# THGLab/NewtonNet

Hardware: AMD Instinct MI355X
Metric: atom-steps/sec (energy+force) on batched MD17 aspirin (higher is better)
Workload: dtype f32; 1 GPU; MD17 aspirin batched inference, 1024 conformers x 21 atoms per GPU, fp32, energy+force, neighbor list included (BASELINE.json configs[1]); 2 independent step(s) in flight per GPU; atoms_per_gpu=21504, weights=seed0, distinct_batches=4, steps_in_flight=2, parallelism=1 independent shard(s), no data-path collective

## Files before the change

### newtonnet_amd/csrc/common.h

```cpp
#pragma once
#include <hip/hip_runtime.h>
#include <stdint.h>

#include "../../include/newtonnet_hip.h"

#if (defined(EDGE_ABL_SELF) || defined(EDGE_ABL_PAIR) || defined(EDGE_ABL_TABLE) || defined(EDGE_ABL_STORE) ||              \
     defined(EDGE_ABL_NO_TABLE) || defined(EDGE_ABL_HALF_TABLE) || defined(EDGE_ABL_NOTAB) || defined(EDGE_ABL_NOMJ) || defined(MLPS_ABL_NO_H) || defined(NS_ABL_NO_Q) || defined(NS_ABL_HOT_W) || defined(MLPS_ABL_X) || defined(ABL_NO_SILU) || defined(ABL_NO_STORE) ||                  \
     (defined(LIN_ABLATE_NO_LOAD) && LIN_ABLATE_NO_LOAD) || (defined(LIN_ABLATE_NO_STORE) && LIN_ABLATE_NO_STORE) ||         \
     (defined(LIN_ABLATE_NO_MFMA) && LIN_ABLATE_NO_MFMA) || (defined(LIN_ABLATE_NO_LDS) && LIN_ABLATE_NO_LDS)) &&            \
    !defined(NNHIP_TOOLING)
#error "ablation switches produce wrong results: build through csrc/build.sh (it marks the library with -DNNHIP_TOOLING)"
#endif

#define NF NNHIP_F
#define NB NNHIP_NB
#define WAVE 64
#ifndef FT_G
#define FT_G 3072
#endif
#define FT_ROWS (FT_G + 8)
#define FT_ZERO_ROW (FT_G + 3)
#define FT_PLANE ((size_t)FT_ROWS * NNHIP_F)

typedef float f32x16 __attribute__((ext_vector_type(16)));
// ... 299 lines not shown
struct WeightImageJobs {
  const float* src[WIMG_MAX_JOBS];
  char* dst[WIMG_MAX_JOBS];
  int fmt;
};
enum { IMG_UPDATE = 0, IMG_NODE0, IMG_NODE2, IMG_UPDATE_T, IMG_NODE0_T, IMG_NODE2_T, IMG_EQ1_0, IMG_EQ1_2, IMG_EQ2_0, IMG_EQ2_2,
       IMG_EQ1_0_T, IMG_EQ1_2_T, IMG_EQ2_0_T, IMG_EQ2_2_T, IMG_PER_LAYER };
enum { IMG_HEAD0 = 0, IMG_HEAD2, IMG_HEAD0_T, IMG_HEAD2_T, IMG_HEAD_COUNT };
struct NodeImages {
  const char *Wu, *W0, *W2;
  const char *W2T, *W0T, *WuT;
};
int launch_weight_images(const float* const* src, char* const* dst, int n, hipStream_t s, int fmt = WIMG_FMT_SPLIT_F16);
int launch_node_fwd_split(const NodeFwdArgs& a, const NodeImages& im, hipStream_t s);
int launch_node_bwd_split(const NodeBwdArgs& a, const NodeImages& im, hipStream_t s);
int launch_mlp_wide_split(int mode, bool accum, const MlpArgs& a, hipStream_t s);
int launch_mlp_wide_pair_split(int mode, const MlpPair& P, hipStream_t s);
int launch_lin_wide_split(const float* X, int ldx, const char* img, float* Y, int ldy, int M, bool acc, hipStream_t s);
bool split_products_enabled();

static inline int cdiv(long a, long b) { return (int)((a + b - 1) / b); }
```

### newtonnet_amd/csrc/edge.hip

```cpp
#include <stdlib.h>

#include <type_traits>

#include "common.h"

#include "edge_common.h"

template <int WPR>
__global__ void __launch_bounds__(64 * EDGE_ROWS)
msg_fwd_kernel(const float* __restrict__ m, const int2* __restrict__ xg, const float* __restrict__ table,
               const int* __restrict__ row_ptr, const int* __restrict__ col, const int* __restrict__ pid,
               const float* __restrict__ a_in, float* __restrict__ msg , float* __restrict__ a_mid,
               int n_atoms) {
  __shared__ float4 comb[EDGE_COMB_SIZE(WPR, 1)];
  int part;
  const int i_ = wave_row_split<WPR>(gridDim.x, part);
  const bool active = i_ < n_atoms;
  if (WPR == 1 && !active) return;
  const int i = active ? i_ : 0;
  const int lane = threadIdx.x & 63;
  const int c4 = 4 * (lane & 31);
  const bool hi = lane >= 32;
  const float4 mi = ld4(m + (size_t)i * NF + c4);
  float4 acc = make_float4(0.f, 0.f, 0.f, 0.f);
// ... 344 lines not shown
      float4 eps, deps;
      filter_value_deriv(table, ABL_G(gx.x), c4, fw, eps, deps);
      const float gxs = half_sum_top(dot4(mul4(mul4(G, mi), mj), deps));
      if ((lane & 31) == 31) g_x[eh] = gxs;
      if (NEED_GM) acc = fma4(mul4(G, eps), mj, acc);
    }
  }
  if (NEED_GM) {
    acc = add4(acc, upper_half(acc));
    float4 a1[1] = {acc};
    row_combine<WPR, 1>(a1, comb, part, lane);
    if (active && part == 0 && !hi) st4(g_m + (size_t)i * NF + c4, a1[0]);
  }
}

template <bool NEED_GM>
__global__ void __launch_bounds__(64 * FM_WAVES)
msg_bwd_mol_kernel(const float* __restrict__ g_msg , const float* __restrict__ g_a, const float* __restrict__ m,
                   const int2* __restrict__ xg, const float* __restrict__ table, const int* __restrict__ mol_ptr,
                   const int* __restrict__ row_ptr, const int* __restrict__ col, const int* __restrict__ pid,
                   float* __restrict__ g_m, float* __restrict__ g_x, int n_mol, const int* __restrict__ pair_ptr) {
  __shared__ __attribute__((aligned(16))) float ml[NNHIP_MOL_STAGE_MAX * NF];
  __shared__ __attribute__((aligned(16))) float gl[NNHIP_MOL_STAGE_MAX * NF];
  __shared__ int s_next;
  const int b = xcd_tile(blockIdx.x, gridDim.x);
  if (b >= n_mol) return;
  const int a0 = mol_ptr[b], n = mol_ptr[b + 1] - a0;
  const bool staged = n <= NNHIP_MOL_STAGE_MAX;
  if (staged) {
    const float4* sm = reinterpret_cast<const float4*>(m + (size_t)a0 * NF);
    const float4* sg = reinterpret_cast<const float4*>(g_a + (size_t)a0 * NF);
    for (int t = threadIdx.x; t < n * (NF / 4); t += 64 * FM_WAVES) {
      reinterpret_cast<float4*>(ml)[t] = sm[t];
      reinterpret_cast<float4*>(gl)[t] = sg[t];
    }
  }
// ... 43 lines not shown
        const float4 mj = node(ml, m, j), gaj = node(gl, g_a, j);
        const float4 G = add4(add4(ld4(g_msg + p * NF + c4), gai), gaj);
        const FilterW fw = filter_weights(__int_as_float(gx.y));
        float4 eps, deps;
        filter_value_deriv(table, gx.x, c4, fw, eps, deps);
        const float gxs = half_sum_top(dot4(mul4(mul4(G, mi), mj), deps));
        if ((lane & 31) == 31) g_x[eh] = gxs;
        if (NEED_GM) acc = fma4(mul4(G, eps), mj, acc);
      }
    }
    if (NEED_GM) {
      acc = add4(acc, upper_half(acc));
      if (!hi) st4(g_m + (size_t)i * NF + c4, acc);
    }
  }
}

__global__ void __launch_bounds__(256)
edge_gd_kernel(const float* __restrict__ g_x , const float* __restrict__ g_u ,
               const float* __restrict__ geo, int n_edges, int n_layers, float inv_rc, float* __restrict__ g_d ) {
  const int e = blockIdx.x * blockDim.x + threadIdx.x;
  if (e >= n_edges) return;
  float gx = 0.f, gu0 = 0.f, gu1 = 0.f, gu2 = 0.f;
  for (int l = 0; l < n_layers; ++l) {
    gx += g_x[(size_t)l * n_edges + e];
    const float4 v = reinterpret_cast<const float4*>(g_u)[(size_t)l * n_edges + e];
    gu0 += v.x;
    gu1 += v.y;
    gu2 += v.z;
  }
// ... 318 lines not shown
  static const size_t v = getenv("NNHIP_EDGE_LDS") ? (size_t)atol(getenv("NNHIP_EDGE_LDS")) : 0;
  return v;
}

static bool mol_kernels_pay(int n_atoms, int n_mol) {
  static const int min_mol = getenv("NNHIP_MOL_KERNELS_MIN") ? atoi(getenv("NNHIP_MOL_KERNELS_MIN")) : 640;
  return n_mol >= min_mol && (long)n_atoms <= (long)n_mol * NNHIP_MOL_STAGE_MAX && (long)n_atoms >= 8L * n_mol;
}

void edge_config(int* small_atoms, int* mol_min, int* wpr , int* mol_forms ) {
  *small_atoms = getenv("NNHIP_EDGE_SMALL_ATOMS") ? atoi(getenv("NNHIP_EDGE_SMALL_ATOMS")) : EDGE_SMALL_ATOMS;
  *mol_min = getenv("NNHIP_MOL_KERNELS_MIN") ? atoi(getenv("NNHIP_MOL_KERNELS_MIN")) : 640;
  wpr[0] = EDGE_WPR_MSG_FWD, wpr[1] = EDGE_WPR_FORCE_FWD, wpr[2] = EDGE_WPR_FORCE_BWD, wpr[3] = EDGE_WPR_MSG_BWD;
  auto off = [](const char* name) { return getenv(name) && atoi(getenv(name)) == 0; };
  *mol_forms = (off("NNHIP_FORCE_FWD_MOL") ? 0 : 1) | (off("NNHIP_MSG_BWD_MOL") ? 0 : 2) | (off("NNHIP_FORCE_DIRECT_MOL") ? 0 : 4) |
               (off("NNHIP_HEAD_OUT_MOL") ? 0 : 8);
}

int launch_msg_fwd(const float* m, const int* xg, const float* table, const int* row_ptr, const int* col,
                   const int* pid, const float* a_in, float* msg, float* a_mid, int n_atoms, hipStream_t s) {
  ScopedTimer t0(TC_EDGE, s);
  ScopedTimer t1(TC_EDGE_FWD_MSG, s);
  EDGE_LAUNCH(msg_fwd_kernel, EDGE_WPR_MSG_FWD, m, reinterpret_cast<const int2*>(xg), table, row_ptr, col, pid, a_in, msg, a_mid, n_atoms);
  LAUNCH_CHECK();
  return 0;
}

int launch_force_fwd(bool has_f, const float* phi1, const float* phi2, const float* geo, const int* row_ptr,
                     const int* col, const int* pid, const float* f_in, float* f_out, int n_atoms, const int* xg,
                     hipStream_t s, const int* pair_ptr, const int* mol_ptr, int n_mol) {
  ScopedTimer t0(TC_EDGE, s);
// ... 18 lines not shown
                     float* g_fin, int n_atoms, const int* xg, hipStream_t s, const int* pair_ptr, const int* rev) {
  ScopedTimer t0(TC_EDGE, s);
  ScopedTimer t1(TC_EDGE_BWD_FORCE, s);
  static const bool owner_off = getenv("NNHIP_FORCE_BWD_OWNER_GU") && atoi(getenv("NNHIP_FORCE_BWD_OWNER_GU")) == 0;
  if (owner_off) rev = nullptr;
  if (has_f)
    EDGE_LAUNCH_B(force_bwd_kernel, true, EDGE_WPR_FORCE_BWD, gf, phi1, phi2, geo, row_ptr, col, pid, f_in, g_h12, g_u, g_fin, n_atoms, reinterpret_cast<const int2*>(xg), pair_ptr, rev);
  else
    EDGE_LAUNCH_B(force_bwd_kernel, false, EDGE_WPR_FORCE_BWD, gf, phi1, phi2, geo, row_ptr, col, pid, f_in, g_h12, g_u, g_fin, n_atoms, reinterpret_cast<const int2*>(xg), pair_ptr, rev);
  LAUNCH_CHECK();
  return 0;
}

int launch_msg_bwd(const float* g_msg, const float* g_a, const float* m, const int* xg, const float* table,
                   const int* row_ptr, const int* col, const int* pid, float* g_m, float* g_x, int n_atoms,
                   bool need_gm, hipStream_t s, const int* pair_ptr, const int* mol_ptr, int n_mol) {
  ScopedTimer t0(TC_EDGE, s);
  ScopedTimer t1(TC_EDGE_BWD_MSG, s);
  static const bool mol_off = getenv("NNHIP_MSG_BWD_MOL") && atoi(getenv("NNHIP_MSG_BWD_MOL")) == 0;
  if (mol_ptr && pair_ptr && mol_kernels_pay(n_atoms, n_mol) && !mol_off) {
    if (need_gm)
      msg_bwd_mol_kernel<true><<<n_mol, 64 * FM_WAVES, 0, s>>>(g_msg, g_a, m, reinterpret_cast<const int2*>(xg), table, mol_ptr, row_ptr,
                                                              col, pid, g_m, g_x, n_mol, pair_ptr);
    else
      msg_bwd_mol_kernel<false><<<n_mol, 64 * FM_WAVES, 0, s>>>(g_msg, g_a, m, reinterpret_cast<const int2*>(xg), table, mol_ptr, row_ptr,
                                                               col, pid, g_m, g_x, n_mol, pair_ptr);
    LAUNCH_CHECK();
    return 0;
  }
  if (need_gm)
    EDGE_LAUNCH_B(msg_bwd_kernel, true, EDGE_WPR_MSG_BWD, g_msg, g_a, m, reinterpret_cast<const int2*>(xg), table, row_ptr, col, pid, g_m, g_x, n_atoms, pair_ptr);
  else
    EDGE_LAUNCH_B(msg_bwd_kernel, false, EDGE_WPR_MSG_BWD, g_msg, g_a, m, reinterpret_cast<const int2*>(xg), table, row_ptr, col, pid, g_m, g_x, n_atoms, pair_ptr);
  LAUNCH_CHECK();
  return 0;
}

#define FD_MAX_EDGES (NNHIP_MOL_STAGE_MAX * (NNHIP_MOL_STAGE_MAX - 1))
__global__ void __launch_bounds__(256)
force_direct_mol_kernel(const float* __restrict__ g_x, const float* __restrict__ g_u, const float* __restrict__ geo,
                        const int* __restrict__ mol_ptr, const int* __restrict__ row_ptr, const int* __restrict__ rev, int n_edges,
// ... 77 lines not shown
                          hipStream_t s) {
  ScopedTimer t0(TC_OTHER, s);
  layer_norm_bwd_kernel<<<cdiv(n_atoms, ROWS_PER_BLOCK), 256, 0, s>>>(g_a, gamma, xhat, rstd, n_atoms);
  LAUNCH_CHECK();
  return 0;
}

int launch_embed(const int64_t* z, const float* table, const float* m_table, int n_atoms, float* a0, float* m0,
                 hipStream_t s) {
  ScopedTimer t0(TC_OTHER, s);
  embed_kernel<<<cdiv((long)n_atoms * (NF / 4), 256), 256, 0, s>>>(z, table, m_table, n_atoms, a0, m0);
  LAUNCH_CHECK();
  return 0;
}

int launch_head_out(const float* e2, const float* w4, const float* b4, const float* scale, const float* shift,
                    const int64_t* z, const int* mol_ptr, int n_atoms, int n_mol, int act, float* atom_energy, float* g_e2,
                    float* energy, hipStream_t s, bool small_molecules) {
  ScopedTimer t0(TC_OTHER, s);
  static const bool mol_off = getenv("NNHIP_HEAD_OUT_MOL") && atoi(getenv("NNHIP_HEAD_OUT_MOL")) == 0;
  if (small_molecules && n_mol > 0 && (long)n_atoms <= (long)n_mol * NNHIP_MOL_STAGE_MAX && !mol_off) {
    head_out_mol_kernel<<<n_mol, 64 * HM_WAVES, 0, s>>>(e2, w4, b4, scale, shift, z, mol_ptr, act, atom_energy, g_e2, energy);
    LAUNCH_CHECK();
    return 0;
  }
  head_out_kernel<<<cdiv(n_atoms, ROWS_PER_BLOCK), 256, 0, s>>>(e2, w4, b4, scale, shift, z, n_atoms, act, atom_energy, g_e2);
  LAUNCH_CHECK();
  const bool big = n_atoms > MOL_SPLIT && n_mol <= 4096 && !small_molecules;
  mol_energy_kernel<<<cdiv(n_mol, ROWS_PER_BLOCK), 256, 0, s>>>(atom_energy, mol_ptr, n_mol, energy, big ? MOL_SPLIT : 0x7fffffff);
  LAUNCH_CHECK();
  if (big) {
    mol_energy_big_kernel<<<n_mol, 1024, 0, s>>>(atom_energy, mol_ptr, n_mol, energy);
    LAUNCH_CHECK();
  }
  return 0;
}

int launch_transposes(const float* const* src, float* const* dst, int count, hipStream_t s) {
  ScopedTimer t0(TC_OTHER, s);
  TransposeList L;
  if (count > 40) return NNHIP_E_INVALID;
  for (int k = 0; k < count; ++k) {
    L.src[k] = src[k];
    L.dst[k] = dst[k];
  }
  transpose128_kernel<<<dim3(NF / 32, NF / 32, count), 256, 0, s>>>(L);
  LAUNCH_CHECK();
  return 0;
}

// ... 50 lines not shown
```

### newtonnet_amd/csrc/node128s.hip

```cpp
#include <stdint.h>
#include <string.h>

#include "common.h"

typedef _Float16 h8 __attribute__((ext_vector_type(8)));
typedef _Float16 h4 __attribute__((ext_vector_type(4)));
typedef __bf16 b8 __attribute__((ext_vector_type(8)));
typedef __bf16 b4 __attribute__((ext_vector_type(4)));

#ifndef NS_WG_PER_CU
#define NS_WG_PER_CU 2
#endif
#define NS_PITCH 272
#define NS_PLANE (32 * NS_PITCH)
#define NS_LDS_BYTES (2 * NS_PLANE + 8 * 32 * 4)
#ifndef NS_MERGE3
#define NS_MERGE3 0
#endif
#define WIMG_PLANE (NF * NF * 2)

__device__ __forceinline__ void ns_pow2_scale(float m, float& S, float& inv) {
  const int e = (int)((__float_as_uint(m) >> 23) & 0xffu);
  const bool ok = e >= 40 && e < 255;
  S = ok ? __uint_as_float((unsigned)(268 - e) << 23) : 1.0f;
// ... 430 lines not shown
    sblk_load(qv, p.q, ((size_t)rc * 3 + c) * NF, t);
#endif
    if (p.G_f) sblk_load(gin, p.G_f, ((size_t)rc * 3 + c) * NF, t);
    tile_gemm_s(out, t, wf, inv);
#pragma unroll
    for (int k = 0; k < 16; ++k) out[k] = fmaf(ga[k], qv[k], out[k]);
    if (p.G_f) {
#pragma unroll
      for (int k = 0; k < 16; ++k) out[k] += gin[k];
    }
    if (live) sblk_store(out, p.gf, ((size_t)row * 3 + c) * NF, t);
  }
#endif
}

__global__ void __launch_bounds__(256, 2) node_tan_fwd_split_kernel(const NodeTanFwdArgs p, const NodeImages im) {
  NS_TILE_SETUP()
  WFrag wf;
  load_wimg(wf, t, im.Wu);
  float upd[16];
#pragma unroll
  for (int k = 0; k < 16; ++k) upd[k] = 0.f;
  float xa[16], xb[16], a[16];
  sblk_load(xa, p.df, ((size_t)rc * 3 + 0) * NF, t);
#pragma unroll
  for (int c = 0; c < 3; ++c) {
    float (&cur)[16] = (c & 1) ? xb : xa;
    float (&nxt)[16] = (c & 1) ? xa : xb;
    float dqv[16], fv[16], qv[16];
    tile_publish(cur, t);
// ... 130 lines not shown
}

int launch_node_fwd_split(const NodeFwdArgs& a, const NodeImages& im, hipStream_t s) {
  if (a.N <= 0) return 0;
  ScopedTimer t0(TC_LIN, s);
  ScopedTimer t1(TC_LIN1, s);
  node_fwd_split_kernel<<<cdiv(a.N, 32), 256, 0, s>>>(a, im);
  LAUNCH_CHECK();
  return 0;
}
int launch_node_bwd_split(const NodeBwdArgs& a, const NodeImages& im, hipStream_t s) {
  if (a.N <= 0) return 0;
  ScopedTimer t0(TC_LIN, s);
  ScopedTimer t1(TC_LIN1, s);
  node_bwd_split_kernel<<<cdiv(a.N, 32), 256, 0, s>>>(a, im);
  LAUNCH_CHECK();
  return 0;
}

template <int MODE>
__device__ __forceinline__ void mlp_wide_split_body(const MlpArgs& p, const bool accum, STile& t) {
  const int M = mlp_rows(p);
  if ((int)blockIdx.x * 32 >= M) return;
  const int row = blockIdx.x * 32 + t.r;
  const int rc = min(row, M - 1);
  const bool live = row < M;

  const bool bf = wimg_is_bf16(p.W1_img);
  WFrag wf;
  load_wimg(wf, t, p.W1_img);
// ... 188 lines not shown
```

### newtonnet_amd/csrc/pipeline.hip

```cpp
#include <stdarg.h>
#include <stdio.h>
#include <string.h>

#include <atomic>
#include <mutex>
#include <vector>

#include "common.h"

int launch_filter_tables(const float* const* edge_w, float* const* tables, int n_layers, const float* freq, int nb,
                         int envelope, hipStream_t s);
int launch_msg_fwd(const float* m, const int* xg, const float* table, const int* row_ptr, const int* col,
                   const int* pid, const float* a_in, float* msg, float* a_mid, int n_atoms, hipStream_t s);
int launch_force_fwd(bool has_f, const float* phi1, const float* phi2, const float* geo, const int* row_ptr,
                     const int* col, const int* pid, const float* f_in, float* f_out, int n_atoms, const int* xg, hipStream_t s,
                     const int* pair_ptr = nullptr, const int* mol_ptr = nullptr, int n_mol = 0);
int launch_force_bwd(bool has_f, const float* gf, const float* phi1, const float* phi2, const float* geo,
                     const int* row_ptr, const int* col, const int* pid, const float* f_in, float* g_h12, float* g_u,
                     float* g_fin, int n_atoms, const int* xg, hipStream_t s, const int* pair_ptr = nullptr, const int* rev = nullptr);
int launch_msg_bwd(const float* g_msg, const float* g_a, const float* m, const int* xg, const float* table,
                   const int* row_ptr, const int* col, const int* pid, float* g_m, float* g_x, int n_atoms, bool need_gm,
                   hipStream_t s, const int* pair_ptr = nullptr, const int* mol_ptr = nullptr, int n_mol = 0);
int launch_geometry_bwd(const float* g_x, const float* g_u, const float* geo, const float* disp, const float* pos,
                        const float* cell, const int* row_ptr, const int* col, const int* rev, const int* mol_ptr,
                        int n_atoms, int n_edges, int n_mol, int n_layers, float cutoff, float* g_d, float* forces,
                        float* virial, hipStream_t s, bool small_molecules = false);
int launch_layer_norm_fwd(float* a, const float* gamma, const float* beta, int n_atoms, float* xhat, float* rstd,
                          hipStream_t s);
int launch_layer_norm_bwd(float* g_a, const float* gamma, const float* xhat, const float* rstd, int n_atoms,
                          hipStream_t s);
int launch_embed(const int64_t* z, const float* table, const float* m_table, int n_atoms, float* a0, float* m0,
                 hipStream_t s);
int launch_head_out(const float* e2, const float* w4, const float* b4, const float* scale, const float* shift,
                    const int64_t* z, const int* mol_ptr, int n_atoms, int n_mol, int act, float* atom_energy, float* g_e2,
                    float* energy, hipStream_t s, bool small_molecules = false);
int launch_transposes(const float* const* src, float* const* dst, int count, hipStream_t s);
static thread_local char g_err[512] = "";
void nnhip_set_error(const char* fmt, ...) {
  va_list ap;
  va_start(ap, fmt);
  vsnprintf(g_err, sizeof(g_err), fmt, ap);
  va_end(ap);
}
extern "C" const char* nnhip_last_error(void) { return g_err; }
extern "C" int nnhip_version(void) { return 113; }
extern "C" int nnhip_build_flags(void) {
#ifdef NNHIP_TOOLING
  return 1;
#else
  return 0;
#endif
}

void edge_config(int* small_atoms, int* mol_min, int* wpr, int* mol_forms);
int mlp_wide_max_tiles_silu();
extern "C" int nnhip_mlp_forms(void);
extern "C" int nnhip_graph_small_max_atoms(void);
extern "C" int nnhip_config(char* buf, size_t n) {
  if (!buf || n < 64) {
    nnhip_set_error("nnhip_config: buffer of at least 64 bytes");
    return NNHIP_E_INVALID;
  }
  static const char* names[] = {"NNHIP_EDGE_LDS", "NNHIP_EDGE_SMALL_ATOMS", "NNHIP_EDGE_WPR", "NNHIP_FORCE_DIRECT_MOL", "NNHIP_FORCE_FWD_MOL", "NNHIP_GRAPH_MOL",
                                "NNHIP_GRAPH_SMALL_ATOMS", "NNHIP_HEAD_OUT_MOL", "NNHIP_MLP_REGW", "NNHIP_MLP_REGW_SINGLE", "NNHIP_MLP_SPLIT",
                                "NNHIP_MLP_WIDE_TILES", "NNHIP_MOL_KERNELS_MIN", "NNHIP_MSG_BWD_MOL",
                                "NNHIP_WGRAD_FORM", "NNHIP_WGRAD_RPC"};
  int small_atoms, mol_min, wpr[4], mol_forms;
  edge_config(&small_atoms, &mol_min, wpr, &mol_forms);
  const int forms = nnhip_mlp_forms();
  const char* graph_mol = getenv("NNHIP_GRAPH_MOL");
  size_t o = 0;
  auto put = [&](const char* fmt, auto... a) {
    if (o < n) {
      const int k = snprintf(buf + o, n - o, fmt, a...);
      o += k > 0 ? (size_t)k : 0;
    }
  };
  put("{\"version\": %d, \"tooling_build\": %d, \"split_f16_products\": %d, ", nnhip_version(), nnhip_build_flags(), forms & 1);
  put("\"neighbor_list\": {\"single_launch_max_atoms\": %d, \"per_molecule_kernels\": %d, \"cell_list\": \"one periodic molecule (host choice)\"}, ",
      nnhip_graph_small_max_atoms(), (graph_mol && atoi(graph_mol) == 0) ? 0 : 1);
  put("\"edge_rows\": {\"waves_per_row\": {\"msg_fwd\": %d, \"force_fwd\": %d, \"force_bwd\": %d, \"msg_bwd\": %d}, \"four_waves_per_row_up_to_atoms\": %d}, ",
      wpr[0], wpr[1], wpr[2], wpr[3], small_atoms);
  put("\"molecule_forms\": {\"max_atoms\": %d, \"edge_kernels_from_molecules\": %d, \"force_fwd\": %d, \"msg_bwd\": %d, \"force_direct\": %d, \"head_out\": %d}, ",
      NNHIP_MOL_STAGE_MAX, mol_min, mol_forms & 1, (mol_forms >> 1) & 1, (mol_forms >> 2) & 1, (mol_forms >> 3) & 1);
  put("\"edge_mlp\": {\"row_local_up_to_tiles\": %d, \"one_pass_adjoint\": %d, \"one_pass_forward\": %d, \"one_pass_single_adjoint\": %d, "
      "\"one_pass_single_forward\": %d}, ",
      mlp_wide_max_tiles_silu(), (forms >> 1) & 1, (forms >> 2) & 1, (forms >> 3) & 1, (forms >> 4) & 1);
  put("\"radial_table_intervals\": %d, \"env\": {", FT_G);
  bool first = true;
  for (const char* nm : names) {
    const char* v = getenv(nm);
    if (!v) continue;
    char clean[25];
    int k = 0;
    for (; k < 24 && v[k]; ++k) {
      const char ch = v[k];
      const bool ok = (ch >= '0' && ch <= '9') || (ch >= 'a' && ch <= 'z') || (ch >= 'A' && ch <= 'Z') || ch == '_' || ch == '.' ||
                      ch == ',' || ch == '+' || ch == '-';
      clean[k] = ok ? ch : '?';
    }
    clean[k] = 0;
    put("%s\"%s\": \"%s\"", first ? "" : ", ", nm, clean);
// ... 517 lines not shown
  char* ws = (char*)workspace;
  auto P = [&](size_t off) { return (float*)(ws + off); };
  const bool want_forces = forces != nullptr;

  PrepLayout pq;
  make_prep_layout(L, pq);
  char* pbase = prepared ? (char*)prepared : ws + w.prep;
  auto Q = [&](size_t off) { return (float*)(pbase + off); };
  if (!prepared) TRY(run_prepare(model, pq, pbase, s));
  const bool split_nodes = split_products_enabled() && act == NNHIP_ACT_SILU;
  if (!embedded) TRY(launch_embed(z, model->node_embedding, Q(pq.m_tab), N, P(w.pub.a0), P(w.pub.m[0]), s));
  const float* a_in = P(w.pub.a0);
  const float* f_in = nullptr;
  auto A_OUT = [&](int l) { return (l == L - 1 && atom_node_out) ? atom_node_out : P(w.pub.a_out[l]); };
  auto F_OUT = [&](int l) { return (l == L - 1 && force_node_out) ? force_node_out : P(w.pub.f_out[l]); };
  for (int l = 0; l < L; ++l) {
    const nnhip_layer_params& lp = model->layer[l];
    const bool has_f = l > 0;
    {
      TRY(launch_msg_fwd(P(w.pub.m[l]), xg, Q(pq.ftab[l]), row_ptr, col, pid, a_in, P(w.pub.msg[l]), P(w.pub.a_mid[l]), N, s));
      if (E > 0) {
        float* h12 = P(w.pub.h12[l]);
        MlpArgs m1 = {P(w.pub.msg[l]), lp.eq1_0_w, lp.eq1_2_w, h12, P(w.pub.phi1[l]), P_, NF, NF, NF};
        MlpArgs m2 = {P(w.pub.msg[l]), lp.eq2_0_w, lp.eq2_2_w, h12 + h2_off, P(w.pub.phi2[l]), P_, NF, NF, NF};
        m1.h_frag = m2.h_frag = 1;
        m1.act = m2.act = act;
        m1.M_dev = m2.M_dev = n_pairs_dev;
        if (split_nodes) {
          m1.W1_img = pbase + pq.img[l][IMG_EQ1_0];
          m1.W2_img = pbase + pq.img[l][IMG_EQ1_2];
          m2.W1_img = pbase + pq.img[l][IMG_EQ2_0];
          m2.W2_img = pbase + pq.img[l][IMG_EQ2_2];
        }
        if (has_f)
          TRY(launch_mlp_pair(MODE_FWD, m1, false, m2, false, s));
        else
          TRY(launch_mlp(MODE_FWD, false, m1, s));
      }
      TRY(launch_force_fwd(has_f, P(w.pub.phi1[l]), P(w.pub.phi2[l]), geo, row_ptr, col, pid, f_in, F_OUT(l), N, mask_xg, s, pair_ptr,
                           mol_kernels ? mol_ptr : nullptr, B));
    }
    {
      NodeFwdArgs na;
      memset(&na, 0, sizeof(na));
      na.f = F_OUT(l);
      na.a_mid = P(w.pub.a_mid[l]);
      na.Wu = lp.update_w;
      na.q = P(w.pub.q[l]);
      na.a_out = A_OUT(l);
      if (l + 1 < L && !lp.ln_w) {
        const nnhip_layer_params& nx = model->layer[l + 1];
        na.W0 = nx.node0_w;
        na.b0 = nx.node0_b;
        na.W2 = nx.node2_w;
        na.b2 = nx.node2_b;
        na.hn = P(w.pub.hn[l + 1]);
        na.m = P(w.pub.m[l + 1]);
// ... 23 lines not shown
    if (lp.ln_w) {
      TRY(launch_layer_norm_fwd(A_OUT(l), lp.ln_w, lp.ln_b, N, P(w.xhat[l]), P(w.rstd[l]), s));
      if (l + 1 < L) {
        const nnhip_layer_params& nx = model->layer[l + 1];
        TRY(launch_mlp(MODE_FWD, false, {A_OUT(l), nx.node0_w, nx.node2_w, P(w.pub.hn[l + 1]), P(w.pub.m[l + 1]), N, NF, NF,
                                         NF, nx.node0_b, nx.node2_b, act}, s));
      }
    }
    a_in = A_OUT(l);
    f_in = F_OUT(l);
  }
  if (model->layer[L - 1].ln_w)
    TRY(launch_mlp(MODE_FWD, false, {a_in, model->head0_w, model->head2_w, P(w.pub.e1), P(w.pub.e2), N, NF, NF, NF,
                                     model->head0_b, model->head2_b, act}, s));
  float* atom_energy = atom_energy_out ? atom_energy_out : P(w.atom_energy);
  TRY(launch_head_out(P(w.pub.e2), model->head4_w, model->head4_b, model->scale, model->shift, z, mol_ptr, N, B,
                      act, atom_energy, want_forces ? P(w.g_e) : nullptr, energy, s, mol_kernels));
  if (!want_forces) return NNHIP_OK;

  auto node_bwd = [&](const NodeBwdArgs& a, const NodeImages& im) {
    return split_nodes ? launch_node_bwd_split(a, im, s) : launch_node_bwd(a, s);
  };
  {
    NodeBwdArgs nb;
    memset(&nb, 0, sizeof(nb));
    nb.g_top = P(w.g_e);
    nb.h_top = P(w.pub.e1);
    nb.W2T = Q(pq.headT[1]);
    nb.W0T = Q(pq.headT[0]);
    nb.g_a = P(w.pub.g_a);
    nb.acc_ga = 0;
    nb.f = F_OUT(L - 1);
    nb.q = P(w.pub.q[L - 1]);
    nb.G_f = nullptr;
    nb.WuT = Q(pq.wT[L - 1][6]);
    nb.gf = P(w.gf_mid);
    nb.N = N;
    nb.act = act;
// ... 2 lines not shown
    bim.W2T = pbase + pq.img_head[IMG_HEAD2_T];
    bim.W0T = pbase + pq.img_head[IMG_HEAD0_T];
    bim.WuT = pbase + pq.img[L - 1][IMG_UPDATE_T];
    const nnhip_layer_params& top = model->layer[L - 1];
    if (top.ln_w) {
      NodeBwdArgs head = nb;
      head.WuT = nullptr;
      TRY(node_bwd(head, bim));
      TRY(launch_layer_norm_bwd(P(w.pub.g_a), top.ln_w, P(w.xhat[L - 1]), P(w.rstd[L - 1]), N, s));
      nb.W2T = nullptr;
    }
    TRY(node_bwd(nb, bim));
  }
  float* g_fbuf[2] = {P(w.pub.g_f), P(w.g_f2)};
  int pp = 0;
  for (int l = L - 1; l >= 0; --l) {
    const nnhip_layer_params& lp = model->layer[l];
    (void)lp;
    const bool has_f = l > 0;
    const float* f_prev = has_f ? F_OUT(l - 1) : nullptr;
    float* g_fin = g_fbuf[pp];
    {
      TRY(launch_force_bwd(has_f, P(w.gf_mid), P(w.pub.phi1[l]), P(w.pub.phi2[l]), geo, row_ptr, col, pid, f_prev,
                           P(w.g_h12), P(w.pub.g_u) + (size_t)l * E * 4, g_fin, N, mask_xg, s, pair_ptr, rev));
      if (E > 0) {
        float* gp = P(w.g_h12);
        float* h12 = P(w.pub.h12[l]);
        MlpArgs m1 = {gp, Q(pq.wT[l][3]), Q(pq.wT[l][2]), h12, P(w.g_msg), P_, 2 * NF, NF, NF};
        MlpArgs m2 = {gp + NF, Q(pq.wT[l][5]), Q(pq.wT[l][4]), h12 + h2_off, P(w.g_msg), P_, 2 * NF, NF, NF};
        m1.h_frag = m2.h_frag = 1;
        m1.act = m2.act = act;
        m1.M_dev = m2.M_dev = n_pairs_dev;
        if (split_nodes) {
          m1.W1_img = pbase + pq.img[l][IMG_EQ1_2_T];
          m1.W2_img = pbase + pq.img[l][IMG_EQ1_0_T];
          m2.W1_img = pbase + pq.img[l][IMG_EQ2_2_T];
          m2.W2_img = pbase + pq.img[l][IMG_EQ2_0_T];
        }
        if (has_f)
          TRY(launch_mlp_pair(MODE_BWD, m1, false, m2, true, s));
        else
          TRY(launch_mlp(MODE_BWD, false, m1, s));
      }
      TRY(launch_msg_bwd(P(w.g_msg), P(w.pub.g_a), P(w.pub.m[l]), xg, Q(pq.ftab[l]), row_ptr, col, pid, P(w.g_m),
                         P(w.pub.g_x) + (size_t)l * E, N, l > 0, s, pair_ptr, mol_kernels ? mol_ptr : nullptr, B));
    }
    if (l > 0) {
      NodeBwdArgs nb;
      memset(&nb, 0, sizeof(nb));
      nb.g_top = P(w.g_m);
      nb.h_top = P(w.pub.hn[l]);
      nb.W2T = Q(pq.wT[l][1]);
      nb.W0T = Q(pq.wT[l][0]);
      nb.g_a = P(w.pub.g_a);
      nb.acc_ga = 1;
      nb.f = F_OUT(l - 1);
      nb.q = P(w.pub.q[l - 1]);
      nb.G_f = g_fin;
      nb.WuT = Q(pq.wT[l - 1][6]);
      nb.gf = P(w.gf_mid);
// ... 4 lines not shown
      bim.W2T = pbase + pq.img[l][IMG_NODE2_T];
      bim.W0T = pbase + pq.img[l][IMG_NODE0_T];
      bim.WuT = pbase + pq.img[l - 1][IMG_UPDATE_T];
      const nnhip_layer_params& below = model->layer[l - 1];
      if (below.ln_w) {
        NodeBwdArgs mlp = nb;
        mlp.WuT = nullptr;
        TRY(node_bwd(mlp, bim));
        TRY(launch_layer_norm_bwd(P(w.pub.g_a), below.ln_w, P(w.xhat[l - 1]), P(w.rstd[l - 1]), N, s));
        nb.W2T = nullptr;
      }
      TRY(node_bwd(nb, bim));
    }
    pp ^= 1;
  }
  TRY(launch_geometry_bwd(P(w.pub.g_x), P(w.pub.g_u), geo, disp, pos, cell, row_ptr, col, rev, mol_ptr, N, E, B, L,
                          model->cutoff, P(w.g_d), forces, virial, s, mol_kernels));
  return NNHIP_OK;
}

extern "C" int nnhip_energy_forces(const nnhip_model* model, const int64_t* z, const float* pos, const float* cell,
                                   const int32_t* mol_ptr, const int32_t* row_ptr, const int32_t* col,
                                   const int32_t* rev, const int32_t* pid, const float* geo, const int32_t* xg,
                                   const float* disp, int32_t N, int32_t E, int32_t B, void* workspace,
                                   size_t workspace_bytes, float* energy, float* forces, float* virial,
                                   float* atom_energy_out, float* atom_node_out, float* force_node_out,
                                   const void* prepared, void* stream_) {
  return energy_forces_impl(model, z, pos, cell, mol_ptr, row_ptr, col, rev, pid, geo, xg, disp, N, E, B, workspace, workspace_bytes,
                            energy, forces, virial, atom_energy_out, atom_node_out, force_node_out, prepared, nullptr, nullptr,
                            stream_);
}
extern "C" int nnhip_energy_forces_pp(const nnhip_model* model, const int64_t* z, const float* pos, const float* cell,
// ... 211 lines not shown
```

### newtonnet_amd/csrc/train_step.hip

```cpp
#include <string.h>

#include "common.h"

int launch_layer_norm_fwd(float* a, const float* gamma, const float* beta, int n_atoms, float* xhat, float* rstd, hipStream_t s);
int launch_layer_norm_bwd(float* g_a, const float* gamma, const float* xhat, const float* rstd, int n_atoms, hipStream_t s);
int launch_layer_norm_tan_fwd(float* da, const float* xhat, const float* rstd, const float* gamma, int n_atoms, float* dxhat,
                              float* drstd, hipStream_t s);
int launch_layer_norm_tan_bwd(const float* gy, float* dga, const float* xhat, const float* rstd, const float* dxhat,
                              const float* drstd, const float* gamma, int n_atoms, float* row_w, float* row_b, hipStream_t s);

int launch_force_fwd(bool has_f, const float* phi1, const float* phi2, const float* geo, const int* row_ptr, const int* col,
                     const int* pid, const float* f_in, float* f_out, int n_atoms, const int* xg, hipStream_t s, const int* pair_ptr,
                     const int* mol_ptr, int n_mol);
int launch_force_bwd(bool has_f, const float* gf, const float* phi1, const float* phi2, const float* geo, const int* row_ptr,
                     const int* col, const int* pid, const float* f_in, float* g_h12, float* g_u, float* g_fin, int n_atoms,
                     const int* xg, hipStream_t s, const int* pair_ptr, const int* rev);
int launch_msg_bwd(const float* g_msg, const float* g_a, const float* m, const int* xg, const float* table, const int* row_ptr,
                   const int* col, const int* pid, float* g_m, float* g_x, int n_atoms, bool need_gm, hipStream_t s,
                   const int* pair_ptr, const int* mol_ptr, int n_mol);

#define TS_TRY(x)          \
  do {                     \
    int _r = (x);          \
    if (_r) return _r;     \
  } while (0)

static nnhip_mlp_desc mlp_desc(int mode, const float* X, int ldx, const float* W1, const float* W2, float* H, float* Y, int M,
                               int act, const void* img1 = nullptr, const void* img2 = nullptr) {
  nnhip_mlp_desc d;
  memset(&d, 0, sizeof(d));
  d.X = X;
  d.ldx = ldx;
  d.W1 = W1;
  d.W2 = W2;
// ... 566 lines not shown
```

Measured before the change: 15.27 million atom-steps/s.

## Fuse last-layer node update with energy head and fold force assembly into msg backward

Adds a node_turn kernel that fuses the last layer's node update, the energy-head MLP forward, per-atom energy, and the head and update backward into one tile kernel. This removes several launches and the global round-trips of e1/e2/g_e. It also appends a force tail to the layer-0 per-molecule msg backward kernel, which computes edge gradients into LDS and reduces them into per-atom forces, replacing the separate geometry backward pass. In exchange, the fused kernels carry more register and LDS pressure and an extra block-level sync phase.

```diff
diff --git a/newtonnet_amd/csrc/common.h b/newtonnet_amd/csrc/common.h
--- a/newtonnet_amd/csrc/common.h
+++ b/newtonnet_amd/csrc/common.h
@@ -337,9 +337,33 @@
 int launch_weight_images(const float* const* src, char* const* dst, int n, hipStream_t s, int fmt = WIMG_FMT_SPLIT_F16);
 int launch_node_fwd_split(const NodeFwdArgs& a, const NodeImages& im, hipStream_t s);
 int launch_node_bwd_split(const NodeBwdArgs& a, const NodeImages& im, hipStream_t s);
+struct NodeTurnArgs {
+  const float* f;
+  const float* a_mid;
+  float* a_out;
+  const float *b0, *b2;
+  const float *w4, *b4;
+  const float *scale, *shift;
+  const int64_t* z;
+  float* atom_energy;
+  float* g_a;
+  float* gf;
+  int N;
+};
+int launch_node_turn_split(const NodeTurnArgs& a, const NodeImages& im, hipStream_t s);
+bool node_turn_enabled();
 int launch_mlp_wide_split(int mode, bool accum, const MlpArgs& a, hipStream_t s);
 int launch_mlp_wide_pair_split(int mode, const MlpPair& P, hipStream_t s);
 int launch_lin_wide_split(const float* X, int ldx, const char* img, float* Y, int ldy, int M, bool acc, hipStream_t s);
 bool split_products_enabled();
 
+struct MsgBwdForceTail {
+  const float* g_u;
+  const float* geo;
+  const int* rev;
+  int n_edges, n_layers;
+  float inv_rc;
+  float* forces;
+};
+
 static inline int cdiv(long a, long b) { return (int)((a + b - 1) / b); }
diff --git a/newtonnet_amd/csrc/edge.hip b/newtonnet_amd/csrc/edge.hip
--- a/newtonnet_amd/csrc/edge.hip
+++ b/newtonnet_amd/csrc/edge.hip
@@ -382,12 +382,16 @@
   }
 }
 
-template <bool NEED_GM>
+__device__ __forceinline__ float4 gd_of_edge(const float* __restrict__ g_x, const float* __restrict__ g_u,
+                                             const float* __restrict__ geo, int e, int n_edges, int n_layers, float inv_rc);
+static_assert((size_t)NNHIP_MOL_STAGE_MAX * (NNHIP_MOL_STAGE_MAX - 1) * sizeof(float4) <= (size_t)NNHIP_MOL_STAGE_MAX * NF * sizeof(float),
+              "g_d of a staged molecule's edges must fit in the LDS rows of m");
+template <bool NEED_GM, bool FORCE>
 __global__ void __launch_bounds__(64 * FM_WAVES)
 msg_bwd_mol_kernel(const float* __restrict__ g_msg , const float* __restrict__ g_a, const float* __restrict__ m,
                    const int2* __restrict__ xg, const float* __restrict__ table, const int* __restrict__ mol_ptr,
                    const int* __restrict__ row_ptr, const int* __restrict__ col, const int* __restrict__ pid,
-                   float* __restrict__ g_m, float* __restrict__ g_x, int n_mol, const int* __restrict__ pair_ptr) {
+                   float* __restrict__ g_m, float* __restrict__ g_x, int n_mol, const int* __restrict__ pair_ptr, const MsgBwdForceTail ft) {
   __shared__ __attribute__((aligned(16))) float ml[NNHIP_MOL_STAGE_MAX * NF];
   __shared__ __attribute__((aligned(16))) float gl[NNHIP_MOL_STAGE_MAX * NF];
   __shared__ int s_next;
@@ -461,6 +465,43 @@
       if (!hi) st4(g_m + (size_t)i * NF + c4, acc);
     }
   }
+  if (FORCE) {
+    __syncthreads();
+    float4* sgd = reinterpret_cast<float4*>(ml);
+    const int E0 = row_ptr[a0];
+    if (staged) {
+      const int nE = row_ptr[a0 + n] - E0;
+      for (int u = threadIdx.x; u < nE; u += 64 * FM_WAVES)
+        sgd[u] = gd_of_edge(g_x, ft.g_u, ft.geo, E0 + u, ft.n_edges, ft.n_layers, ft.inv_rc);
+    }
+    __syncthreads();
+    const int sub = threadIdx.x & 15;
+    for (int k0 = 0; k0 < n; k0 += 4 * FM_WAVES) {
+      const int k = k0 + (threadIdx.x >> 4);
+      const int i = a0 + k;
+      float fx = 0.f, fy = 0.f, fz = 0.f;
+      if (k < n) {
+        for (int e = row_ptr[i] + sub; e < row_ptr[i + 1]; e += 16) {
+          const float4 a = staged ? sgd[e - E0] : gd_of_edge(g_x, ft.g_u, ft.geo, e, ft.n_edges, ft.n_layers, ft.inv_rc);
+          const float4 c = staged ? sgd[ft.rev[e] - E0] : gd_of_edge(g_x, ft.g_u, ft.geo, ft.rev[e], ft.n_edges, ft.n_layers, ft.inv_rc);
+          fx -= (a.x - c.x);
+          fy -= (a.y - c.y);
+          fz -= (a.z - c.z);
+        }
+      }
+#pragma unroll
+      for (int o = 8; o > 0; o >>= 1) {
+        fx += __shfl_xor(fx, o, WAVE);
+        fy += __shfl_xor(fy, o, WAVE);
+        fz += __shfl_xor(fz, o, WAVE);
+      }
+      if (k < n && sub == 0) {
+        ft.forces[3 * (size_t)i] = fx;
+        ft.forces[3 * (size_t)i + 1] = fy;
+        ft.forces[3 * (size_t)i + 2] = fz;
+      }
+    }
+  }
 }
 
 __global__ void __launch_bounds__(256)
@@ -809,7 +850,8 @@
   wpr[0] = EDGE_WPR_MSG_FWD, wpr[1] = EDGE_WPR_FORCE_FWD, wpr[2] = EDGE_WPR_FORCE_BWD, wpr[3] = EDGE_WPR_MSG_BWD;
   auto off = [](const char* name) { return getenv(name) && atoi(getenv(name)) == 0; };
   *mol_forms = (off("NNHIP_FORCE_FWD_MOL") ? 0 : 1) | (off("NNHIP_MSG_BWD_MOL") ? 0 : 2) | (off("NNHIP_FORCE_DIRECT_MOL") ? 0 : 4) |
-               (off("NNHIP_HEAD_OUT_MOL") ? 0 : 8);
+               (off("NNHIP_HEAD_OUT_MOL") ? 0 : 8) |
+               ((off("NNHIP_MSG_BWD_FORCE") || off("NNHIP_MSG_BWD_MOL") || off("NNHIP_FORCE_DIRECT_MOL")) ? 0 : 16);
 }
 
 int launch_msg_fwd(const float* m, const int* xg, const float* table, const int* row_ptr, const int* col,
@@ -858,17 +900,26 @@
 
 int launch_msg_bwd(const float* g_msg, const float* g_a, const float* m, const int* xg, const float* table,
                    const int* row_ptr, const int* col, const int* pid, float* g_m, float* g_x, int n_atoms,
-                   bool need_gm, hipStream_t s, const int* pair_ptr, const int* mol_ptr, int n_mol) {
+                   bool need_gm, hipStream_t s, const int* pair_ptr, const int* mol_ptr, int n_mol, const MsgBwdForceTail* tail,
+                   bool* tail_done) {
   ScopedTimer t0(TC_EDGE, s);
   ScopedTimer t1(TC_EDGE_BWD_MSG, s);
+  if (tail_done) *tail_done = false;
   static const bool mol_off = getenv("NNHIP_MSG_BWD_MOL") && atoi(getenv("NNHIP_MSG_BWD_MOL")) == 0;
   if (mol_ptr && pair_ptr && mol_kernels_pay(n_atoms, n_mol) && !mol_off) {
+    const MsgBwdForceTail none = {};
+    static const bool tail_off = (getenv("NNHIP_MSG_BWD_FORCE") && atoi(getenv("NNHIP_MSG_BWD_FORCE")) == 0) ||
+                                 (getenv("NNHIP_FORCE_DIRECT_MOL") && atoi(getenv("NNHIP_FORCE_DIRECT_MOL")) == 0);
     if (need_gm)
-      msg_bwd_mol_kernel<true><<<n_mol, 64 * FM_WAVES, 0, s>>>(g_msg, g_a, m, reinterpret_cast<const int2*>(xg), table, mol_ptr, row_ptr,
-                                                              col, pid, g_m, g_x, n_mol, pair_ptr);
-    else
-      msg_bwd_mol_kernel<false><<<n_mol, 64 * FM_WAVES, 0, s>>>(g_msg, g_a, m, reinterpret_cast<const int2*>(xg), table, mol_ptr, row_ptr,
-                                                               col, pid, g_m, g_x, n_mol, pair_ptr);
+      msg_bwd_mol_kernel<true, false><<<n_mol, 64 * FM_WAVES, 0, s>>>(g_msg, g_a, m, reinterpret_cast<const int2*>(xg), table, mol_ptr,
+                                                                     row_ptr, col, pid, g_m, g_x, n_mol, pair_ptr, none);
+    else if (tail && tail_done && !tail_off) {
+      msg_bwd_mol_kernel<false, true><<<n_mol, 64 * FM_WAVES, 0, s>>>(g_msg, g_a, m, reinterpret_cast<const int2*>(xg), table, mol_ptr,
+                                                                     row_ptr, col, pid, g_m, g_x, n_mol, pair_ptr, *tail);
+      *tail_done = true;
+    } else
+      msg_bwd_mol_kernel<false, false><<<n_mol, 64 * FM_WAVES, 0, s>>>(g_msg, g_a, m, reinterpret_cast<const int2*>(xg), table, mol_ptr,
+                                                                      row_ptr, col, pid, g_m, g_x, n_mol, pair_ptr, none);
     LAUNCH_CHECK();
     return 0;
   }
@@ -976,6 +1027,17 @@
   return 0;
 }
 
+static int mol_energy_sums(const float* atom_energy, const int* mol_ptr, int n_atoms, int n_mol, float* energy, hipStream_t s,
+                           bool small_molecules) {
+  const bool big = n_atoms > MOL_SPLIT && n_mol <= 4096 && !small_molecules;
+  mol_energy_kernel<<<cdiv(n_mol, ROWS_PER_BLOCK), 256, 0, s>>>(atom_energy, mol_ptr, n_mol, energy, big ? MOL_SPLIT : 0x7fffffff);
+  LAUNCH_CHECK();
+  if (big) {
+    mol_energy_big_kernel<<<n_mol, 1024, 0, s>>>(atom_energy, mol_ptr, n_mol, energy);
+    LAUNCH_CHECK();
+  }
+  return 0;
+}
 int launch_head_out(const float* e2, const float* w4, const float* b4, const float* scale, const float* shift,
                     const int64_t* z, const int* mol_ptr, int n_atoms, int n_mol, int act, float* atom_energy, float* g_e2,
                     float* energy, hipStream_t s, bool small_molecules) {
@@ -988,14 +1050,12 @@
   }
   head_out_kernel<<<cdiv(n_atoms, ROWS_PER_BLOCK), 256, 0, s>>>(e2, w4, b4, scale, shift, z, n_atoms, act, atom_energy, g_e2);
   LAUNCH_CHECK();
-  const bool big = n_atoms > MOL_SPLIT && n_mol <= 4096 && !small_molecules;
-  mol_energy_kernel<<<cdiv(n_mol, ROWS_PER_BLOCK), 256, 0, s>>>(atom_energy, mol_ptr, n_mol, energy, big ? MOL_SPLIT : 0x7fffffff);
-  LAUNCH_CHECK();
-  if (big) {
-    mol_energy_big_kernel<<<n_mol, 1024, 0, s>>>(atom_energy, mol_ptr, n_mol, energy);
-    LAUNCH_CHECK();
-  }
-  return 0;
+  return mol_energy_sums(atom_energy, mol_ptr, n_atoms, n_mol, energy, s, small_molecules);
+}
+int launch_mol_energy(const float* atom_energy, const int* mol_ptr, int n_atoms, int n_mol, float* energy, hipStream_t s,
+                      bool small_molecules) {
+  ScopedTimer t0(TC_OTHER, s);
+  return mol_energy_sums(atom_energy, mol_ptr, n_atoms, n_mol, energy, s, small_molecules);
 }
 
 int launch_transposes(const float* const* src, float* const* dst, int count, hipStream_t s) {
diff --git a/newtonnet_amd/csrc/node128s.hip b/newtonnet_amd/csrc/node128s.hip
--- a/newtonnet_amd/csrc/node128s.hip
+++ b/newtonnet_amd/csrc/node128s.hip
@@ -468,6 +468,125 @@
 #endif
 }
 
+#define NT_PITCH 132
+static_assert(32 * NT_PITCH * 4 <= 2 * NS_PLANE, "the fp32 e2 tile must fit in the f16 planes of the LDS tile");
+__global__ void __launch_bounds__(256, NS_WG_PER_CU_BWD) node_turn_split_kernel(const NodeTurnArgs p, const NodeImages im) {
+  NS_TILE_SETUP()
+  WFrag wf;
+  load_wimg(wf, t, im.Wu);
+  float fk[3][16], qk[3][16], a[16];
+  {
+    float upd[16];
+#pragma unroll
+    for (int k = 0; k < 16; ++k) upd[k] = 0.f;
+    sblk_load(fk[0], p.f, ((size_t)rc * 3 + 0) * NF, t);
+#pragma unroll
+    for (int c = 0; c < 3; ++c) {
+      tile_publish(fk[c], t);
+      __syncthreads();
+      const float inv = tile_commit(fk[c], t);
+      __syncthreads();
+      if (c < 2)
+        sblk_load(fk[c + 1], p.f, ((size_t)rc * 3 + c + 1) * NF, t);
+      else
+        sblk_load(a, p.a_mid, (size_t)rc * NF, t);
+      tile_gemm_s(qk[c], t, wf, inv);
+      if (c == 2) load_wimg(wf, t, im.W0);
+#pragma unroll
+      for (int k = 0; k < 16; ++k) upd[k] = fmaf(fk[c][k], qk[c][k], upd[k]);
+    }
+#pragma unroll
+    for (int k = 0; k < 16; ++k) a[k] += upd[k];
+  }
+  if (live) sblk_store(a, p.a_out, (size_t)row * NF, t);
+
+  tile_publish(a, t);
+  __syncthreads();
+  float inv = tile_commit(a, t);
+  __syncthreads();
+  float e1[16], v[16], bv[16];
+  sblk_load(bv, p.b0, 0, t);
+  tile_gemm_s(e1, t, wf, inv);
+  load_wimg(wf, t, im.W2);
+#pragma unroll
+  for (int k = 0; k < 16; ++k) e1[k] += bv[k];
+#pragma unroll
+  for (int k = 0; k < 16; ++k) v[k] = silu_f(e1[k]);
+  tile_publish(v, t);
+  __syncthreads();
+  inv = tile_commit(v, t);
+  __syncthreads();
+  sblk_load(bv, p.b2, 0, t);
+  float e2[16];
+  tile_gemm_s(e2, t, wf, inv);
+  load_wimg(wf, t, im.W2T);
+#pragma unroll
+  for (int k = 0; k < 16; ++k) e2[k] += bv[k];
+
+  float* et = reinterpret_cast<float*>(lds);
+  __syncthreads();
+  {
+    float4* er = reinterpret_cast<float4*>(et + t.r * NT_PITCH + t.nb * 32 + 4 * t.h);
+#pragma unroll
+    for (int q = 0; q < 4; ++q) er[2 * q] = make_float4(e2[4 * q], e2[4 * q + 1], e2[4 * q + 2], e2[4 * q + 3]);
+  }
+  __syncthreads();
+  {
+    const int lane = threadIdx.x & 63;
+    const float2 w = ld2(p.w4 + 2 * lane);
+    for (int j = 0; j < 8; ++j) {
+      const int rr = t.nb * 8 + j;
+      const int i = blockIdx.x * 32 + rr;
+      if (i >= p.N) break;
+      const float2 h = *reinterpret_cast<const float2*>(et + rr * NT_PITCH + 2 * lane);
+      const float ax = silu_f(h.x), ay = silu_f(h.y);
+      const float s = wave_sum(fmaf(ax, w.x, ay * w.y));
+      const long zi = clamp_species(p.z[i]);
+      const float sc = p.scale ? p.scale[zi] : 1.0f;
+      const float sh = p.shift ? p.shift[zi] : 0.0f;
+      if (lane == 0) p.atom_energy[i] = fmaf(s + p.b4[0], sc, sh);
+    }
+  }
+  {
+    const float sc = p.scale ? p.scale[clamp_species(p.z[rc])] : 1.0f;
+    sblk_load(bv, p.w4, 0, t);
+#pragma unroll
+    for (int k = 0; k < 16; ++k) v[k] = sc * bv[k] * dsilu_f(e2[k]);
+  }
+
+  float ga[16];
+  tile_publish(v, t);
+  __syncthreads();
+  inv = tile_commit(v, t);
+  __syncthreads();
+  tile_gemm_s(v, t, wf, inv);
+  load_wimg(wf, t, im.W0T);
+#pragma unroll
+  for (int k = 0; k < 16; ++k) v[k] *= dsilu_f(e1[k]);
+  tile_publish(v, t);
+  __syncthreads();
+  inv = tile_commit(v, t);
+  __syncthreads();
+  tile_gemm_s(ga, t, wf, inv);
+  load_wimg(wf, t, im.WuT);
+  if (live) sblk_store(ga, p.g_a, (size_t)row * NF, t);
+
+#pragma unroll
+  for (int c = 0; c < 3; ++c) {
+    float out[16];
+#pragma unroll
+    for (int k = 0; k < 16; ++k) fk[c][k] *= ga[k];
+    tile_publish(fk[c], t);
+    __syncthreads();
+    inv = tile_commit(fk[c], t);
+    __syncthreads();
+    tile_gemm_s(out, t, wf, inv);
+#pragma unroll
+    for (int k = 0; k < 16; ++k) out[k] = fmaf(ga[k], qk[c][k], out[k]);
+    if (live) sblk_store(out, p.gf, ((size_t)row * 3 + c) * NF, t);
+  }
+}
+
 __global__ void __launch_bounds__(256, 2) node_tan_fwd_split_kernel(const NodeTanFwdArgs p, const NodeImages im) {
   NS_TILE_SETUP()
   WFrag wf;
@@ -628,6 +747,19 @@
   ScopedTimer t0(TC_LIN, s);
   ScopedTimer t1(TC_LIN1, s);
   node_bwd_split_kernel<<<cdiv(a.N, 32), 256, 0, s>>>(a, im);
+  LAUNCH_CHECK();
+  return 0;
+}
+
+bool node_turn_enabled() {
+  static const bool on = !(getenv("NNHIP_NODE_TURN") && atoi(getenv("NNHIP_NODE_TURN")) == 0);
+  return on;
+}
+int launch_node_turn_split(const NodeTurnArgs& a, const NodeImages& im, hipStream_t s) {
+  if (a.N <= 0) return 0;
+  ScopedTimer t0(TC_LIN, s);
+  ScopedTimer t1(TC_LIN1, s);
+  node_turn_split_kernel<<<cdiv(a.N, 32), 256, 0, s>>>(a, im);
   LAUNCH_CHECK();
   return 0;
 }
diff --git a/newtonnet_amd/csrc/pipeline.hip b/newtonnet_amd/csrc/pipeline.hip
--- a/newtonnet_amd/csrc/pipeline.hip
+++ b/newtonnet_amd/csrc/pipeline.hip
@@ -20,7 +20,8 @@
                      float* g_fin, int n_atoms, const int* xg, hipStream_t s, const int* pair_ptr = nullptr, const int* rev = nullptr);
 int launch_msg_bwd(const float* g_msg, const float* g_a, const float* m, const int* xg, const float* table,
                    const int* row_ptr, const int* col, const int* pid, float* g_m, float* g_x, int n_atoms, bool need_gm,
-                   hipStream_t s, const int* pair_ptr = nullptr, const int* mol_ptr = nullptr, int n_mol = 0);
+                   hipStream_t s, const int* pair_ptr = nullptr, const int* mol_ptr = nullptr, int n_mol = 0,
+                   const MsgBwdForceTail* tail = nullptr, bool* tail_done = nullptr);
 int launch_geometry_bwd(const float* g_x, const float* g_u, const float* geo, const float* disp, const float* pos,
                         const float* cell, const int* row_ptr, const int* col, const int* rev, const int* mol_ptr,
                         int n_atoms, int n_edges, int n_mol, int n_layers, float cutoff, float* g_d, float* forces,
@@ -34,6 +35,8 @@
 int launch_head_out(const float* e2, const float* w4, const float* b4, const float* scale, const float* shift,
                     const int64_t* z, const int* mol_ptr, int n_atoms, int n_mol, int act, float* atom_energy, float* g_e2,
                     float* energy, hipStream_t s, bool small_molecules = false);
+int launch_mol_energy(const float* atom_energy, const int* mol_ptr, int n_atoms, int n_mol, float* energy, hipStream_t s,
+                      bool small_molecules = false);
 int launch_transposes(const float* const* src, float* const* dst, int count, hipStream_t s);
 static thread_local char g_err[512] = "";
 void nnhip_set_error(const char* fmt, ...) {
@@ -63,7 +66,7 @@
   }
   static const char* names[] = {"NNHIP_EDGE_LDS", "NNHIP_EDGE_SMALL_ATOMS", "NNHIP_EDGE_WPR", "NNHIP_FORCE_DIRECT_MOL", "NNHIP_FORCE_FWD_MOL", "NNHIP_GRAPH_MOL",
                                 "NNHIP_GRAPH_SMALL_ATOMS", "NNHIP_HEAD_OUT_MOL", "NNHIP_MLP_REGW", "NNHIP_MLP_REGW_SINGLE", "NNHIP_MLP_SPLIT",
-                                "NNHIP_MLP_WIDE_TILES", "NNHIP_MOL_KERNELS_MIN", "NNHIP_MSG_BWD_MOL",
+                                "NNHIP_MLP_WIDE_TILES", "NNHIP_MOL_KERNELS_MIN", "NNHIP_MSG_BWD_FORCE", "NNHIP_MSG_BWD_MOL", "NNHIP_NODE_TURN",
                                 "NNHIP_WGRAD_FORM", "NNHIP_WGRAD_RPC"};
   int small_atoms, mol_min, wpr[4], mol_forms;
   edge_config(&small_atoms, &mol_min, wpr, &mol_forms);
@@ -81,11 +84,13 @@
       nnhip_graph_small_max_atoms(), (graph_mol && atoi(graph_mol) == 0) ? 0 : 1);
   put("\"edge_rows\": {\"waves_per_row\": {\"msg_fwd\": %d, \"force_fwd\": %d, \"force_bwd\": %d, \"msg_bwd\": %d}, \"four_waves_per_row_up_to_atoms\": %d}, ",
       wpr[0], wpr[1], wpr[2], wpr[3], small_atoms);
-  put("\"molecule_forms\": {\"max_atoms\": %d, \"edge_kernels_from_molecules\": %d, \"force_fwd\": %d, \"msg_bwd\": %d, \"force_direct\": %d, \"head_out\": %d}, ",
-      NNHIP_MOL_STAGE_MAX, mol_min, mol_forms & 1, (mol_forms >> 1) & 1, (mol_forms >> 2) & 1, (mol_forms >> 3) & 1);
+  put("\"molecule_forms\": {\"max_atoms\": %d, \"edge_kernels_from_molecules\": %d, \"force_fwd\": %d, \"msg_bwd\": %d, \"force_direct\": %d, \"head_out\": %d, "
+      "\"msg_bwd_with_forces\": %d}, ",
+      NNHIP_MOL_STAGE_MAX, mol_min, mol_forms & 1, (mol_forms >> 1) & 1, (mol_forms >> 2) & 1, (mol_forms >> 3) & 1, (mol_forms >> 4) & 1);
   put("\"edge_mlp\": {\"row_local_up_to_tiles\": %d, \"one_pass_adjoint\": %d, \"one_pass_forward\": %d, \"one_pass_single_adjoint\": %d, "
       "\"one_pass_single_forward\": %d}, ",
       mlp_wide_max_tiles_silu(), (forms >> 1) & 1, (forms >> 2) & 1, (forms >> 3) & 1, (forms >> 4) & 1);
+  put("\"node_turn_fused\": %d, ", ((forms & 1) && node_turn_enabled()) ? 1 : 0);
   put("\"radial_table_intervals\": %d, \"env\": {", FT_G);
   bool first = true;
   for (const char* nm : names) {
@@ -633,6 +638,7 @@
   const float* f_in = nullptr;
   auto A_OUT = [&](int l) { return (l == L - 1 && atom_node_out) ? atom_node_out : P(w.pub.a_out[l]); };
   auto F_OUT = [&](int l) { return (l == L - 1 && force_node_out) ? force_node_out : P(w.pub.f_out[l]); };
+  const bool node_turn = split_nodes && want_forces && !model->layer[L - 1].ln_w && node_turn_enabled();
   for (int l = 0; l < L; ++l) {
     const nnhip_layer_params& lp = model->layer[l];
     const bool has_f = l > 0;
@@ -659,7 +665,7 @@
       TRY(launch_force_fwd(has_f, P(w.pub.phi1[l]), P(w.pub.phi2[l]), geo, row_ptr, col, pid, f_in, F_OUT(l), N, mask_xg, s, pair_ptr,
                            mol_kernels ? mol_ptr : nullptr, B));
     }
-    {
+    if (!(node_turn && l == L - 1)) {
       NodeFwdArgs na;
       memset(&na, 0, sizeof(na));
       na.f = F_OUT(l);
@@ -713,14 +719,43 @@
     TRY(launch_mlp(MODE_FWD, false, {a_in, model->head0_w, model->head2_w, P(w.pub.e1), P(w.pub.e2), N, NF, NF, NF,
                                      model->head0_b, model->head2_b, act}, s));
   float* atom_energy = atom_energy_out ? atom_energy_out : P(w.atom_energy);
-  TRY(launch_head_out(P(w.pub.e2), model->head4_w, model->head4_b, model->scale, model->shift, z, mol_ptr, N, B,
-                      act, atom_energy, want_forces ? P(w.g_e) : nullptr, energy, s, mol_kernels));
+  if (node_turn) {
+    NodeTurnArgs nt;
+    memset(&nt, 0, sizeof(nt));
+    nt.f = F_OUT(L - 1);
+    nt.a_mid = P(w.pub.a_mid[L - 1]);
+    nt.a_out = A_OUT(L - 1);
+    nt.b0 = model->head0_b;
+    nt.b2 = model->head2_b;
+    nt.w4 = model->head4_w;
+    nt.b4 = model->head4_b;
+    nt.scale = model->scale;
+    nt.shift = model->shift;
+    nt.z = z;
+    nt.atom_energy = atom_energy;
+    nt.g_a = P(w.pub.g_a);
+    nt.gf = P(w.gf_mid);
+    nt.N = N;
+    NodeImages im;
+    memset(&im, 0, sizeof(im));
+    im.Wu = pbase + pq.img[L - 1][IMG_UPDATE];
+    im.W0 = pbase + pq.img_head[IMG_HEAD0];
+    im.W2 = pbase + pq.img_head[IMG_HEAD2];
+    im.W2T = pbase + pq.img_head[IMG_HEAD2_T];
+    im.W0T = pbase + pq.img_head[IMG_HEAD0_T];
+    im.WuT = pbase + pq.img[L - 1][IMG_UPDATE_T];
+    TRY(launch_node_turn_split(nt, im, s));
+    TRY(launch_mol_energy(atom_energy, mol_ptr, N, B, energy, s, mol_kernels));
+  } else {
+    TRY(launch_head_out(P(w.pub.e2), model->head4_w, model->head4_b, model->scale, model->shift, z, mol_ptr, N, B,
+                        act, atom_energy, want_forces ? P(w.g_e) : nullptr, energy, s, mol_kernels));
+  }
   if (!want_forces) return NNHIP_OK;
 
   auto node_bwd = [&](const NodeBwdArgs& a, const NodeImages& im) {
     return split_nodes ? launch_node_bwd_split(a, im, s) : launch_node_bwd(a, s);
   };
-  {
+  if (!node_turn) {
     NodeBwdArgs nb;
     memset(&nb, 0, sizeof(nb));
     nb.g_top = P(w.g_e);
@@ -753,6 +788,9 @@
   }
   float* g_fbuf[2] = {P(w.pub.g_f), P(w.g_f2)};
   int pp = 0;
+  MsgBwdForceTail ftail = {P(w.pub.g_u), geo, rev, E, L, 1.0f / model->cutoff, forces};
+  const bool ftail_ok = mol_kernels && !virial && B > 0 && (long)N <= (long)B * NNHIP_MOL_STAGE_MAX;
+  bool forces_done = false;
   for (int l = L - 1; l >= 0; --l) {
     const nnhip_layer_params& lp = model->layer[l];
     (void)lp;
@@ -782,7 +820,8 @@
           TRY(launch_mlp(MODE_BWD, false, m1, s));
       }
       TRY(launch_msg_bwd(P(w.g_msg), P(w.pub.g_a), P(w.pub.m[l]), xg, Q(pq.ftab[l]), row_ptr, col, pid, P(w.g_m),
-                         P(w.pub.g_x) + (size_t)l * E, N, l > 0, s, pair_ptr, mol_kernels ? mol_ptr : nullptr, B));
+                         P(w.pub.g_x) + (size_t)l * E, N, l > 0, s, pair_ptr, mol_kernels ? mol_ptr : nullptr, B,
+                         (l == 0 && ftail_ok) ? &ftail : nullptr, &forces_done));
     }
     if (l > 0) {
       NodeBwdArgs nb;
@@ -817,8 +856,9 @@
     }
     pp ^= 1;
   }
-  TRY(launch_geometry_bwd(P(w.pub.g_x), P(w.pub.g_u), geo, disp, pos, cell, row_ptr, col, rev, mol_ptr, N, E, B, L,
-                          model->cutoff, P(w.g_d), forces, virial, s, mol_kernels));
+  if (!forces_done)
+    TRY(launch_geometry_bwd(P(w.pub.g_x), P(w.pub.g_u), geo, disp, pos, cell, row_ptr, col, rev, mol_ptr, N, E, B, L,
+                            model->cutoff, P(w.g_d), forces, virial, s, mol_kernels));
   return NNHIP_OK;
 }
 
diff --git a/newtonnet_amd/csrc/train_step.hip b/newtonnet_amd/csrc/train_step.hip
--- a/newtonnet_amd/csrc/train_step.hip
+++ b/newtonnet_amd/csrc/train_step.hip
@@ -17,7 +17,7 @@
                      const int* xg, hipStream_t s, const int* pair_ptr, const int* rev);
 int launch_msg_bwd(const float* g_msg, const float* g_a, const float* m, const int* xg, const float* table, const int* row_ptr,
                    const int* col, const int* pid, float* g_m, float* g_x, int n_atoms, bool need_gm, hipStream_t s,
-                   const int* pair_ptr, const int* mol_ptr, int n_mol);
+                   const int* pair_ptr, const int* mol_ptr, int n_mol, const MsgBwdForceTail* tail = nullptr, bool* tail_done = nullptr);
 
 #define TS_TRY(x)          \
   do {                     \
```

Result: faster. 15.53 million atom-steps/s (median of 6 runs) (+1.7%).
